# KyanChen/RSPrompter

Measured on AMD Instinct MI355X. Metric: images/sec (1024x1024 synthetic tiles, rsprompter_anchor SAM-ViT-H, full predict path), higher is better.
Workload: dtype f32 (fp32 in/out; GEMMs and attention as fp16x3 split-precision MFMA with fp32 accumulate); 1 GPU; rsprompter_anchor SAM-ViT-huge, batch 8x1024x1024 per GPU, 10 classes, seeded synthetic weights (the per-GPU slice of BASELINE.json configs[3] on 1 GPU); parallelism=single GPU

## Files before the change

### include/rsp_hip.h

```cpp
#ifndef RSP_HIP_H_
#define RSP_HIP_H_

#include <stdint.h>

#ifdef __cplusplus
extern "C" {
#endif

#define RSP_OK 0
#define RSP_EINVAL (-1)
#define RSP_ELAUNCH (-2)

#define RSP_ACT_NONE 0
#define RSP_ACT_RELU 1
#define RSP_ACT_GELU 2
#define RSP_ACT_SIGMOID 3
#define RSP_ACT_RELU_POST 4

typedef void* rsp_stream_t;

int rsp_abi_version(void);
const char* rsp_build_info(void);

#define RSP_PLANE_F8 0x100
// ... 100 lines not shown
  int64_t k_bs, k_ts, k_hs;
  int64_t v_bs, v_ts, v_hs;
  int64_t o_bs, o_ts, o_hs;
  int32_t B, nh, dh, Tq, Tk;
  float scale;
  uint16_t* out_hi; uint16_t* out_lo; int32_t out_scale_log2;
  const uint8_t* mask;
} RspAttnDesc;
int rsp_attention(const RspAttnDesc* desc, rsp_stream_t stream);

int rsp_sam_t2i_attention(const float* q, const float* kv, const int32_t* kv_map, float* out, int32_t R, int32_t T,
                          int32_t N, float scale, rsp_stream_t stream);
int rsp_sam_i2t_attention(const float* q, const int32_t* q_map, const float* k, const float* v, float* out,
                          uint16_t* out_hi, uint16_t* out_lo, int32_t out_scale_log2, int32_t R, int32_t T, int32_t N,
                          float scale, rsp_stream_t stream);
typedef struct RspI2tFusedDesc {
  const float* q; const int32_t* q_map; const float* k; const float* v;
  const float* wo; const float* bo;
  const float* res; const int32_t* res_map;
  const uint16_t* res_hi; const uint16_t* res_lo; int32_t res_scale_log2;
  const float* gamma; const float* beta; float eps;
  float* out; uint16_t* out_hi; uint16_t* out_lo; int32_t out_scale_log2;
  int32_t R, T, N; float scale;
} RspI2tFusedDesc;
int rsp_sam_i2t_fused(const RspI2tFusedDesc* desc, rsp_stream_t stream);

typedef struct RspRoiAlignDesc {
  const float* feat[4];
  const float* pe[4];
  int32_t H[4], W[4];
  float spatial_scale[4];
  const float* rois;
  float* out;
  int32_t K, P, C, num_levels, finest_scale;
} RspRoiAlignDesc;
int rsp_roi_align(const RspRoiAlignDesc* desc, rsp_stream_t stream);

typedef struct RspBoxCoder {
  float means[4], stds[4];
  float max_ratio;
  float ctr_clamp;
  int32_t clip_border;
  int32_t add_ctr_clamp;
} RspBoxCoder;
typedef struct RspRpnDesc {
  const float* head[5];
// ... 163 lines not shown
```

### rsprompter_amd/_lib.py

```python
import ctypes
import os

_HERE = os.path.dirname(os.path.abspath(__file__))
LIB_PATH = os.path.join(_HERE, "librsp_hip.so")

c_void_p = ctypes.c_void_p
c_int = ctypes.c_int
c_int64 = ctypes.c_int64
c_float = ctypes.c_float


class RspGemmDesc(ctypes.Structure):
    _fields_ = [
        ("A", c_void_p), ("Bhi", c_void_p), ("Blo", c_void_p), ("C", c_void_p),
        ("bias", c_void_p), ("res", c_void_p), ("a_rowmap", c_void_p), ("c_rowmap", c_void_p),
        ("M", c_int), ("N", c_int), ("K", c_int),
        ("lda", c_int), ("ldc", c_int), ("ldr", c_int),
        ("res_mod", c_int), ("act", c_int),
        ("alpha", c_float), ("a_scale_log2", c_int),
        ("conv_k", c_int), ("conv_stride", c_int), ("conv_pad", c_int),
        ("conv_H", c_int), ("conv_W", c_int), ("conv_C", c_int),
        ("conv_Ho", c_int), ("conv_Wo", c_int),
        ("ct_W", c_int), ("ct_dy", c_int),
        ("res_bmap", c_void_p), ("res_brows", c_int),
# ... 14 lines not shown
        ("q_bs", c_int64), ("q_ts", c_int64), ("q_hs", c_int64),
        ("k_bs", c_int64), ("k_ts", c_int64), ("k_hs", c_int64),
        ("v_bs", c_int64), ("v_ts", c_int64), ("v_hs", c_int64),
        ("o_bs", c_int64), ("o_ts", c_int64), ("o_hs", c_int64),
        ("B", c_int), ("nh", c_int), ("dh", c_int), ("Tq", c_int), ("Tk", c_int),
        ("scale", c_float),
        ("out_hi", c_void_p), ("out_lo", c_void_p), ("out_scale_log2", c_int),
        ("mask", c_void_p),
    ]


class RspMaskEmbedDesc(ctypes.Structure):
    _fields_ = [(n, c_void_p) for n in (
        "mask_pred_plus", "image_embeddings", "roi_img", "conv1_w", "conv1_b", "ln1_w", "ln1_b", "conv2_w",
        "conv2_b", "ln2_w", "ln2_b", "conv3_w", "conv3_b", "out")] + [
        ("R", c_int), ("he", c_int), ("we", c_int), ("C", c_int), ("eps", c_float)]


class RspI2tFusedDesc(ctypes.Structure):
    _fields_ = [("q", c_void_p), ("q_map", c_void_p), ("k", c_void_p), ("v", c_void_p), ("wo", c_void_p), ("bo", c_void_p),
                ("res", c_void_p), ("res_map", c_void_p), ("res_hi", c_void_p), ("res_lo", c_void_p),
                ("res_scale_log2", c_int), ("gamma", c_void_p), ("beta", c_void_p), ("eps", c_float),
                ("out", c_void_p), ("out_hi", c_void_p), ("out_lo", c_void_p), ("out_scale_log2", c_int),
                ("R", c_int), ("T", c_int), ("N", c_int), ("scale", c_float)]


class RspRoiAlignDesc(ctypes.Structure):
    _fields_ = [
        ("feat", c_void_p * 4), ("pe", c_void_p * 4), ("H", c_int * 4), ("W", c_int * 4),
        ("spatial_scale", c_float * 4), ("rois", c_void_p), ("out", c_void_p),
        ("K", c_int), ("P", c_int), ("C", c_int), ("num_levels", c_int), ("finest_scale", c_int),
    ]


class RspBoxCoder(ctypes.Structure):
    _fields_ = [("means", c_float * 4), ("stds", c_float * 4), ("max_ratio", c_float), ("ctr_clamp", c_float),
                ("clip_border", c_int), ("add_ctr_clamp", c_int)]


class RspRpnDesc(ctypes.Structure):
    _fields_ = [
        ("head", c_void_p * 5), ("H", c_int * 5), ("W", c_int * 5), ("stride", c_float * 5),
        ("ld", c_int), ("A", c_int), ("nms_pre", c_int), ("num_levels", c_int),
        ("base_anchors", c_void_p), ("coder", RspBoxCoder), ("min_bbox_size", c_float),
    ]


# ... 155 lines not shown
```

### rsprompter_amd/csrc/samattn.hip

```cpp
#include <stdlib.h>
#include "rsp_common.h"

namespace {

constexpr int NH = 8, DH = 16, W = NH * DH;
constexpr float LOG2E = 1.4426950408889634f;

template <int TMAX>
__global__ __launch_bounds__(512) void sam_t2i_kernel(const float* __restrict__ q, const float* __restrict__ kv,
                                                      const int32_t* __restrict__ kv_map, float* __restrict__ out,
                                                      int T, int N, float scale) {
  constexpr int HD = DH / 2;
  __shared__ __attribute__((aligned(16))) float sQ[TMAX * W];
  const int r = blockIdx.x;
  const int tid = threadIdx.x, lane = tid & 63;
  const int h = __builtin_amdgcn_readfirstlane(tid >> 6);
  const int half = lane & 1;
  for (int i = tid; i < TMAX * W; i += 512)
    sQ[i] = (i < T * W) ? q[(int64_t)r * T * W + i] * (scale * LOG2E) : 0.f;
  __syncthreads();
  const int64_t rb = kv_map ? kv_map[r] : r;
  const float* kbase = kv + rb * (int64_t)N * (2 * W) + h * DH + half * HD;
  const float* qbase = &sQ[h * DH + half * HD];

// ... 132 lines not shown
      if (out) *reinterpret_cast<f32x4*>(out + orow * W + h * DH + 4 * c) = o[c];
      if (ohi) {
        half4_t h4, l4;
#pragma unroll
        for (int e = 0; e < 4; ++e) { half_t a, b; rsp_split1(o[c][e] * pscale, a, b); h4[e] = a; l4[e] = b; }
        const int col = h * DH + 4 * c;
        const int64_t po = ((int64_t)(col >> 5) * out_rows + orow) * 32 + (col & 31);
        *reinterpret_cast<half4_t*>(ohi + po) = h4;
        *reinterpret_cast<half4_t*>(olo + po) = l4;
      }
    }
  }
}


struct I2tFusedP {
  const float* q; const int32_t* q_map; const float* k; const float* v;
  const float* wo; const float* bo;
  const float* res; const int32_t* res_map;
  const half_t* res_hi; const half_t* res_lo; float res_inv_scale; int64_t res_rows;
  const float* gamma; const float* beta; float eps;
  float* out; half_t* ohi; half_t* olo; float pscale; int64_t out_rows;
  int T, N; float scale;
};
constexpr int FUSED_PIX_PER_BLOCK = 512, CO = 256;

template <int TMAX>
__global__ __launch_bounds__(1024) void sam_i2t_fused_kernel(const I2tFusedP p) {
  constexpr int PST = TMAX * NH + 8;
  __shared__ __attribute__((aligned(16))) float sK[TMAX * W];
  __shared__ __attribute__((aligned(16))) float sV[TMAX * W];
  __shared__ __attribute__((aligned(16))) float sVp[TMAX * NH * CO];
  __shared__ __attribute__((aligned(16))) float sP[128 * PST];
  __shared__ __attribute__((aligned(16))) float sBo[CO], sG[CO], sB[CO];
  const int r = blockIdx.y;
  const int tid = threadIdx.x;
  const int T = p.T, N = p.N;
  if (tid < CO) { sBo[tid] = p.bo[tid]; sG[tid] = p.gamma[tid]; sB[tid] = p.beta[tid]; }
  for (int i = tid; i < TMAX * W; i += 1024) {
    const bool ok = i < T * W;
    sK[i] = ok ? p.k[(int64_t)r * T * W + i] * (p.scale * LOG2E) : 0.f;
    sV[i] = ok ? p.v[(int64_t)r * T * W + i] : 0.f;
  }
  __syncthreads();
  for (int i = tid; i < TMAX * NH * CO; i += 1024) {
    const int c = i & (CO - 1), th = i >> 8, h = th & 7, t = th >> 3;
// ... 89 lines not shown
    for (int j = 0; j < 8; ++j)
#pragma unroll
      for (int e = 0; e < 4; ++e) { const float dl = acc[j][e] - mean; sq += dl * dl; }
    sq += __shfl_xor(sq, 1, 64); sq += __shfl_xor(sq, 2, 64); sq += __shfl_xor(sq, 4, 64);
    const float rstd = 1.0f / sqrtf(sq * (1.0f / CO) + p.eps);
    if (!live) continue;
#pragma unroll
    for (int j = 0; j < 8; ++j) {
      f32x4 o;
      const f32x4 g4 = *reinterpret_cast<const f32x4*>(&sG[32 * j + 4 * l8]);
      const f32x4 b4 = *reinterpret_cast<const f32x4*>(&sB[32 * j + 4 * l8]);
#pragma unroll
      for (int e = 0; e < 4; ++e) o[e] = (acc[j][e] - mean) * rstd * g4[e] + b4[e];
      if (p.out) *reinterpret_cast<f32x4*>(p.out + orow * CO + 32 * j + 4 * l8) = o;
      if (p.ohi) rsp_store_planes4(p.ohi, p.olo, ((int64_t)j * p.out_rows + orow) * 32 + 4 * l8, o * p.pscale, false);
    }
  }
}


constexpr int F2_THREADS = 512, F2_RPOS = 256, F2_POS = 1024;
typedef float f32x16_t __attribute__((ext_vector_type(16)));

template <int NKS, bool RES_F32>
__global__ __launch_bounds__(F2_THREADS) void sam_i2t_fused_mfma_kernel(const I2tFusedP p) {
  constexpr int TT = 2 * NKS;
  constexpr int TBR = 272, TBW = 32 * TBR, PGB = NKS * 2 * 1024;
  constexpr int REG = PGB > TBW ? PGB : TBW;
  __shared__ __attribute__((aligned(1024))) unsigned char smem[8 * REG + (2 * TT * W + 3 * CO + 2 * 8 * 8 * 32 + 16) * 4];
  float* const sK = reinterpret_cast<float*>(smem + 8 * REG);
  float* const sV = sK + TT * W;
  float* const sBo = sV + TT * W;
  float* const sG = sBo + CO;
  float* const sB = sG + CO;
  float* const sSum = sB + CO;
  float* const sSq = sSum + 8 * 8 * 32;
  float* const sRed = sSq + 8 * 8 * 32;
  const int r = blockIdx.y;
  const int tid = threadIdx.x, lane = tid & 63;
  const int wave = __builtin_amdgcn_readfirstlane(tid >> 6);
  const int hh = lane >> 5, l31 = lane & 31;
  const int T = p.T, N = p.N;
  if (tid < CO) { sBo[tid] = p.bo[tid]; sG[tid] = p.gamma[tid]; sB[tid] = p.beta[tid]; }
  for (int i = tid; i < TT * W; i += F2_THREADS) {
    const bool ok = i < T * W;
    sK[i] = ok ? p.k[(int64_t)r * T * W + i] * (p.scale * LOG2E) : 0.f;
    sV[i] = ok ? p.v[(int64_t)r * T * W + i] : 0.f;
  }
  __syncthreads();
  half8_t ah[NKS], al[NKS];
  float unscale;
  {
    float vp[NKS][8];
// ... 19 lines not shown
    }
    vmax = rsp_wave_max(vmax);
    if (lane == 0) sRed[wave] = vmax;
    __syncthreads();
    float bm = sRed[0];
#pragma unroll
    for (int w = 1; w < 8; ++w) bm = fmaxf(bm, sRed[w]);
    int ve = 0;
    if (bm > 0.f) { int ex; frexpf(bm, &ex); ve = 13 - ex; }
    ve = max(-24, min(24, ve));
    const float vs = ldexpf(1.0f, ve);
    unscale = ldexpf(1.0f, -(14 + ve));
#pragma unroll
    for (int s_ = 0; s_ < NKS; ++s_)
#pragma unroll
      for (int h = 0; h < 8; ++h) {
        half_t a, b;
        rsp_split1(vp[s_][h] * vs, a, b);
        ah[s_][h] = a; al[s_][h] = b;
      }
  }
  const int64_t qb = p.q_map ? p.q_map[r] : r;
  const int64_t rb = p.res_map ? p.res_map[r] : r;
  unsigned char* const piece = smem + wave * REG;
  const int p_blk = blockIdx.x * F2_POS;
  const int lr0 = lane >> 4, c4 = (lane & 15) * 4;
  const int ch0 = wave * 32 + 4 * hh;

  for (int rd = 0; rd < F2_POS / F2_RPOS; ++rd) {
    const int p_round = p_blk + rd * F2_RPOS;
    if (p_round >= N) break;
    asm volatile("" ::: "memory");
    {
      const int p_base = p_round + wave * 32;
      unsigned char* const tb_row = piece + lr0 * TBR + c4 * 4;
      unsigned char* const tb_pos = piece + l31 * TBR;
      float sc[NKS][8];
#pragma unroll
      for (int half = 0; half < 2; ++half) {
#pragma unroll
        for (int g = 0; g < 8; ++g) {
          const int pos = min(p_base + g * 4 + lr0, N - 1);
          const f32x4 x = *reinterpret_cast<const f32x4*>(p.q + (qb * N + pos) * (int64_t)W + half * 64 + c4);
          *reinterpret_cast<f32x4*>(tb_row + g * 4 * TBR) = x;
        }
        RSP_WAVE_LOCKSTEP();
#pragma unroll
        for (int hl = 0; hl < 4; ++hl) {
          const int h = half * 4 + hl;
          f32x4 qv[4];
#pragma unroll
          for (int u = 0; u < 4; ++u) qv[u] = *reinterpret_cast<const f32x4*>(tb_pos + (hl * 4 + u) * 16);
#pragma unroll
          for (int tt = 0; tt < NKS; ++tt) {
            const float* kr = sK + (2 * tt + hh) * W + h * DH;
            f32x2 a2 = {0.f, 0.f};
// ... 12 lines not shown
#pragma unroll
      for (int h = 0; h < 8; ++h) {
        float m = sc[0][h];
#pragma unroll
        for (int tt = 1; tt < NKS; ++tt) m = fmaxf(m, sc[tt][h]);
        m = fmaxf(m, __shfl_xor(m, 32, 64));
        float sm = 0.f;
#pragma unroll
        for (int tt = 0; tt < NKS; ++tt) { sc[tt][h] = __builtin_amdgcn_exp2f(sc[tt][h] - m); sm += sc[tt][h]; }
        sm += __shfl_xor(sm, 32, 64);
        const float inv = 16384.0f / sm;
#pragma unroll
        for (int tt = 0; tt < NKS; ++tt) sc[tt][h] *= inv;
      }
#pragma unroll
      for (int tt = 0; tt < NKS; ++tt) {
        half8_t ph, pl;
        rsp_split8_trunc(sc[tt], ph, pl);
        *reinterpret_cast<half8_t*>(piece + (tt * 2 + 0) * 1024 + lane * 16) = ph;
        *reinterpret_cast<half8_t*>(piece + (tt * 2 + 1) * 1024 + lane * 16) = pl;
      }
    }
    __syncthreads();
#pragma unroll 1
    for (int g0 = 0; g0 < 8; g0 += 4) {
    f32x16_t acc[4];
#pragma unroll
    for (int gl = 0; gl < 4; ++gl) {
      const int g = g0 + gl;
#pragma unroll
      for (int e = 0; e < 16; ++e) acc[gl][e] = 0.f;
#pragma unroll
      for (int s_ = 0; s_ < NKS; ++s_) {
        const half8_t bh = *reinterpret_cast<const half8_t*>(smem + g * REG + (s_ * 2 + 0) * 1024 + lane * 16);
        const half8_t bl = *reinterpret_cast<const half8_t*>(smem + g * REG + (s_ * 2 + 1) * 1024 + lane * 16);
        acc[gl] = __builtin_amdgcn_mfma_f32_32x32x16_f16(al[s_], bh, acc[gl], 0, 0, 0);
        acc[gl] = __builtin_amdgcn_mfma_f32_32x32x16_f16(ah[s_], bl, acc[gl], 0, 0, 0);
        acc[gl] = __builtin_amdgcn_mfma_f32_32x32x16_f16(ah[s_], bh, acc[gl], 0, 0, 0);
      }
      __builtin_amdgcn_sched_barrier(0);
    }
    f32x4 rf[2][4];
    half4_t rh[2][4], rl[2][4];
    auto res_load = [&](int g, int b) {
      const int pos = min(p_round + g * 32 + l31, N - 1);
      if constexpr (RES_F32) {
        const float* rp = p.res + (rb * N + pos) * (int64_t)CO + ch0;
#pragma unroll
        for (int a = 0; a < 4; ++a) rf[b][a] = *reinterpret_cast<const f32x4*>(rp + 8 * a);
      } else {
        const int64_t ro = ((int64_t)wave * p.res_rows + (int64_t)r * N + pos) * 32 + 4 * hh;
#pragma unroll
        for (int a = 0; a < 4; ++a) {
          rh[b][a] = *reinterpret_cast<const half4_t*>(p.res_hi + ro + 8 * a);
          rl[b][a] = *reinterpret_cast<const half4_t*>(p.res_lo + ro + 8 * a);
        }
      }
    };
// ... 81 lines not shown
}

extern "C" int rsp_sam_i2t_attention(const float* q, const int32_t* q_map, const float* k, const float* v, float* out,
                                     uint16_t* out_hi, uint16_t* out_lo, int32_t out_scale_log2, int32_t R, int32_t T,
                                     int32_t N, float scale, rsp_stream_t stream) {
  if (!q || !k || !v || (!out && !(out_hi && out_lo)) || R < 0 || T <= 0 || T > 16 || N <= 0) return RSP_EINVAL;
  if ((out_hi == nullptr) != (out_lo == nullptr)) return RSP_EINVAL;
  if (R == 0) return RSP_OK;
  if (R > 65535) return RSP_EINVAL;
  hipStream_t s = (hipStream_t)stream;
  dim3 grid((N + PIX_PER_BLOCK - 1) / PIX_PER_BLOCK, R);
  half_t* hi = reinterpret_cast<half_t*>(out_hi);
  half_t* lo = reinterpret_cast<half_t*>(out_lo);
  const float ps = ldexpf(1.0f, out_scale_log2);
  const int64_t rows = (int64_t)R * N;
  if (T <= 8) hipLaunchKernelGGL((sam_i2t_kernel<8>), grid, dim3(256), 0, s, q, q_map, k, v, out, hi, lo, ps, T, N, rows, scale);
  else if (T <= 12) hipLaunchKernelGGL((sam_i2t_kernel<12>), grid, dim3(256), 0, s, q, q_map, k, v, out, hi, lo, ps, T, N, rows, scale);
  else hipLaunchKernelGGL((sam_i2t_kernel<16>), grid, dim3(256), 0, s, q, q_map, k, v, out, hi, lo, ps, T, N, rows, scale);
  RSP_CHECK_LAUNCH();
  return RSP_OK;
}

extern "C" int rsp_sam_i2t_fused(const RspI2tFusedDesc* d, rsp_stream_t stream) {
  if (!d || !d->q || !d->k || !d->v || !d->wo || !d->bo || !d->gamma || !d->beta) return RSP_EINVAL;
  if (!d->out && !(d->out_hi && d->out_lo)) return RSP_EINVAL;
  if ((d->out_hi == nullptr) != (d->out_lo == nullptr)) return RSP_EINVAL;
  if ((d->res != nullptr) == (d->res_hi != nullptr) || (d->res_hi && !d->res_lo)) return RSP_EINVAL;
  if (d->R < 0 || d->T <= 0 || d->T > 10 || d->N <= 0 || d->R > 65535) return RSP_EINVAL;
  if (RSP_PLANE_IS_F8(d->out_scale_log2) || RSP_PLANE_IS_F8(d->res_scale_log2)) return RSP_EINVAL;
  if (d->R == 0) return RSP_OK;
  I2tFusedP p;
  p.q = d->q; p.q_map = d->q_map; p.k = d->k; p.v = d->v; p.wo = d->wo; p.bo = d->bo;
  p.res = d->res; p.res_map = d->res_map;
  p.res_hi = reinterpret_cast<const half_t*>(d->res_hi); p.res_lo = reinterpret_cast<const half_t*>(d->res_lo);
  p.res_inv_scale = ldexpf(1.0f, -RSP_PLANE_EXP(d->res_scale_log2)); p.res_rows = (int64_t)d->R * d->N;
  p.gamma = d->gamma; p.beta = d->beta; p.eps = d->eps;
  p.out = d->out; p.ohi = reinterpret_cast<half_t*>(d->out_hi); p.olo = reinterpret_cast<half_t*>(d->out_lo);
  p.pscale = ldexpf(1.0f, RSP_PLANE_EXP(d->out_scale_log2)); p.out_rows = (int64_t)d->R * d->N;
  p.T = d->T; p.N = d->N; p.scale = d->scale;
  hipStream_t s = (hipStream_t)stream;
  const bool mfma_form = !d->out;
  if (mfma_form) {
    dim3 grid2((d->N + F2_POS - 1) / F2_POS, d->R);
    const bool f32res = d->res != nullptr;
    if (d->T <= 8) {
      if (f32res) hipLaunchKernelGGL((sam_i2t_fused_mfma_kernel<4, true>), grid2, dim3(F2_THREADS), 0, s, p);
      else hipLaunchKernelGGL((sam_i2t_fused_mfma_kernel<4, false>), grid2, dim3(F2_THREADS), 0, s, p);
    } else {
      if (f32res) hipLaunchKernelGGL((sam_i2t_fused_mfma_kernel<5, true>), grid2, dim3(F2_THREADS), 0, s, p);
      else hipLaunchKernelGGL((sam_i2t_fused_mfma_kernel<5, false>), grid2, dim3(F2_THREADS), 0, s, p);
    }
    RSP_CHECK_LAUNCH();
    return RSP_OK;
  }
  dim3 grid((d->N + FUSED_PIX_PER_BLOCK - 1) / FUSED_PIX_PER_BLOCK, d->R);
  if (d->T <= 8) hipLaunchKernelGGL((sam_i2t_fused_kernel<8>), grid, dim3(1024), 0, s, p);
  else hipLaunchKernelGGL((sam_i2t_fused_kernel<10>), grid, dim3(1024), 0, s, p);
  RSP_CHECK_LAUNCH();
  return RSP_OK;
}
```

### rsprompter_amd/ops.py

```python
import math
import os

import torch

from . import _lib as _lib_real

ACT_NONE, ACT_RELU, ACT_GELU, ACT_SIGMOID, ACT_RELU_POST = 0, 1, 2, 3, 4
DEFAULT_A_SCALE_LOG2 = 2
DEBUG_FINITE = bool(int(__import__('os').environ.get('RSP_DEBUG_FINITE', '0')))


class Profiler:

    def __init__(self):
        self.records = []

    def summary(self):
        torch.cuda.synchronize()
        agg = {}
        for name, flops, nbytes, e0, e1 in self.records:
            a = agg.setdefault(name, dict(ms=0.0, calls=0, flops=0.0, bytes=0.0))
            a['ms'] += e0.elapsed_time(e1)
            a['calls'] += 1
            a['flops'] += flops
# ... 393 lines not shown


def vit_window_attention(q, kv, rel_tab, Bp, nh, dh, scale, planes=False, f8=False, win_grid=None, variant=0):
    lib = _lib.load()
    T, D = 196, nh * dh
    if not isinstance(kv, Planes) or kv.shape[-1] != 2 * D or kv.rows < Bp * T or kv.f8:
        raise ValueError('kv must be the fp16 K | V planes of the qkv GEMM')
    if tuple(rel_tab.shape) != (2, 2, 32, dh + 8) or rel_tab.dtype != torch.float16 or not rel_tab.is_contiguous():
        raise ValueError('rel_tab must come from pack_relpos_tables')
    _chk_f32(q, 'q')
    out = None if planes else torch.empty((Bp * T, D), dtype=torch.float32, device=q.device)
    pl = empty_planes((Bp * T, D), q.device, f8=f8) if planes else None
    hi, lo, e = (pl.hi.data_ptr(), pl.lo.data_ptr(), pl.word) if planes else (0, 0, 0)
    wn, wr = (int(win_grid[0]), int(win_grid[1])) if win_grid is not None else (0, 0)
    _timed('attn_win_kernel<vit,window>', 4.0 * Bp * nh * T * T * dh, 0,
           lambda: _lib.check(lib.rsp_vit_window_attention(q.data_ptr(), q.stride(0), kv.hi.data_ptr(), kv.lo.data_ptr(),
                                                           kv.rows, kv.scale_log2, rel_tab.data_ptr(), _ptr(out), hi, lo, e,
                                                           Bp, nh, dh, scale, wn, wr, variant, _stream()),
                              'rsp_vit_window_attention'))
    return pl if planes else out


SAM_I2T_FUSED_MAX_TOKENS = 10


def sam_i2t_fused(q, k, v, wo, bo, gamma, beta, *, R, T, N, scale, eps=1e-6, q_map=None, res=None, res_map=None,
                  res_planes=None, planes=True, f32=False):
    lib = _lib.load()
    for t, n in ((q, 'q'), (k, 'k'), (v, 'v'), (wo, 'wo'), (bo, 'bo'), (gamma, 'gamma'), (beta, 'beta')):
        _chk_f32(t, n)
        if not t.is_contiguous():
            raise ValueError(f'sam_i2t_fused: {n} must be contiguous')
    if tuple(wo.shape) != (256, 128) or q.shape[-1] != 128:
        raise ValueError('sam_i2t_fused expects internal width 128 and a [256, 128] out_proj weight')
    if (res is None) == (res_planes is None):
        raise ValueError('sam_i2t_fused: exactly one of res / res_planes')
    d = _lib.RspI2tFusedDesc()
    d.q, d.q_map, d.k, d.v, d.wo, d.bo = q.data_ptr(), _ptr(q_map), k.data_ptr(), v.data_ptr(), wo.data_ptr(), bo.data_ptr()
    if res is not None:
        _chk_f32(res, 'res')
        if not res.is_contiguous() or res.shape[-1] != 256:
            raise ValueError('sam_i2t_fused: res must be contiguous rows of 256')
        d.res, d.res_map = res.data_ptr(), _ptr(res_map)
    else:
        if res_planes.f8 or res_planes.rows != R * N or res_planes.shape[-1] != 256:
            raise ValueError('sam_i2t_fused: res_planes must be the fp16 hi / lo planes of the [R*N, 256] tensor')
        d.res_hi, d.res_lo, d.res_scale_log2 = res_planes.hi.data_ptr(), res_planes.lo.data_ptr(), res_planes.scale_log2
    d.gamma, d.beta, d.eps = gamma.data_ptr(), beta.data_ptr(), eps
    out = torch.empty((R * N, 256), dtype=torch.float32, device=q.device) if f32 else None
    pl = empty_planes((R * N, 256), q.device) if planes else None
    d.out = _ptr(out)
    if pl is not None:
        d.out_hi, d.out_lo, d.out_scale_log2 = pl.hi.data_ptr(), pl.lo.data_ptr(), pl.scale_log2
    d.R, d.T, d.N, d.scale = R, T, N, scale
    _timed('sam_i2t_fused_kernel', 2.0 * R * N * T * (128 + 8 * 256), 4.0 * R * N * (128 + 256 + 256),
           lambda: _lib.check(lib.rsp_sam_i2t_fused(d, _stream()), "rsp_sam_i2t_fused"), detail=f'R={R} T={T} N={N}')
    if planes and f32:
        return out, pl
    return pl if planes else out


_attn_ws = {}


def _attn_workspace(nbytes, device):
    key = str(device)
    buf = _attn_ws.get(key)
    if buf is None or buf.numel() < nbytes:
        buf = torch.empty((nbytes,), dtype=torch.uint8, device=device)
        _attn_ws[key] = buf
    return buf


def vit_attention(qkv, rel, Bp, S, nh, dh, scale, planes=False):
    lib = _lib.load()
    kind = 'global' if S * S >= 1024 else 'window'
    fl = 4.0 * Bp * nh * (S * S) ** 2 * dh
    pl = empty_planes((Bp * S * S, nh * dh), qkv.device) if planes else None
# ... 912 lines not shown
```

### rsprompter_amd/sam_decoder.py

```python
import math

import numpy as np
import torch

from . import ops
from .nnutil import HIPModule, add_param, infer_sam_arch, nchw_view, nhwc_view
from .registry import MODELS

HID = 256
HEADS = 8
MLP_DIM = 2048
N_MASK_TOKENS = 4


def _upscale2_k_order():
    return [32 * ((kp >> 4) >> 1) + 8 * ((8 * ((kp >> 4) & 1) + (kp & 7)) >> 2) + 4 * ((kp >> 3) & 1) + (kp & 3) for kp in range(64)]


def _add_linear(root, name, cout, cin):
    add_param(root, name + '.weight', (cout, cin))
    add_param(root, name + '.bias', (cout,))


def _add_ln(root, name, c):
# ... 26 lines not shown
            _add_attn(self, p + '.cross_attn_image_to_token', HID // 2)
            for j in range(1, 5):
                _add_ln(self, f'{p}.layer_norm{j}', HID)
            _add_linear(self, p + '.mlp.lin1', MLP_DIM, HID)
            _add_linear(self, p + '.mlp.lin2', HID, MLP_DIM)
        _add_attn(self, 'transformer.final_attn_token_to_image', HID // 2)
        _add_ln(self, 'transformer.layer_norm_final_attn', HID)
        add_param(self, 'upscale_conv1.weight', (HID, HID // 4, 2, 2))
        add_param(self, 'upscale_conv1.bias', (HID // 4,))
        add_param(self, 'upscale_conv2.weight', (HID // 4, HID // 8, 2, 2))
        add_param(self, 'upscale_conv2.bias', (HID // 8,))
        _add_ln(self, 'upscale_layer_norm', HID // 4)
        for i in range(N_MASK_TOKENS):
            p = f'output_hypernetworks_mlps.{i}'
            _add_linear(self, p + '.proj_in', HID, HID)
            _add_linear(self, p + '.layers.0', HID, HID)
            _add_linear(self, p + '.proj_out', HID // 8, HID)
        _add_linear(self, 'iou_prediction_head.proj_in', HID, HID)
        _add_linear(self, 'iou_prediction_head.layers.0', HID, HID)
        _add_linear(self, 'iou_prediction_head.proj_out', N_MASK_TOKENS, HID)
        self._pe_cache = {}
        self.t2i_fold = True
        self.upscale_fused = True
        self.keep_stages = False
        self._last_stages = None
        self.max_prompt_sets = None

    def _pw(self, name, with_bias=True):
        m = _g(self, name)
        return ops.PackedWeight(m.weight, m.bias if with_bias else None)

    def _pack(self):
        from .necks import convt_weights4
        P = {}
        for i in range(2):
            p = f'transformer.layers.{i}'
            for a in ('self_attn', 'cross_attn_token_to_image', 'cross_attn_image_to_token'):
                for pr in ('q_proj', 'k_proj', 'v_proj', 'out_proj'):
                    P[f'{i}.{a}.{pr}'] = self._pw(f'{p}.{a}.{pr}')
            P[f'{i}.lin1'] = self._pw(p + '.mlp.lin1')
            P[f'{i}.lin2'] = self._pw(p + '.mlp.lin2')
        for pr in ('q_proj', 'k_proj', 'v_proj', 'out_proj'):
            P[f'final.{pr}'] = self._pw(f'transformer.final_attn_token_to_image.{pr}')
        P['up1'] = convt_weights4(self.upscale_conv1.weight, self.upscale_conv1.bias)
        P['up2'] = convt_weights4(self.upscale_conv2.weight, self.upscale_conv2.bias)
        w2 = self.upscale_conv2.weight.detach()[_upscale2_k_order()]
# ... 165 lines not shown
            keys_pl = ops.layernorm(keys, m4.weight, m4.bias, 1e-6, planes=True, f32=False)
            del keys
        del qi, kv_img

        qpe = ops.add_rows(q, tokens0)
        q = self._token_attn(qpe, qpe, q, '1.self_attn', R, T, res=q)
        q = self._ln(q, 'transformer.layers.1.layer_norm1')
        qpe = ops.add_rows(q, tokens0)
        tq = ops.gemm(qpe, P['1.cross_attn_token_to_image.q_proj'])
        fold = self.t2i_fold and T <= ops.SAM_T2I_FOLD_MAX_TOKENS and N % 32 == 0 and R * N * 512 < 2 ** 31
        kv = None
        if fold:
            ao = self._t2i_folded('1.cross_attn_token_to_image', tq, keys_pl, pe_t, R, T, N)
        else:
            kv = ops.gemm(keys_pl, P['1.cross_attn_token_to_image.kv_proj'], bias=None,
                          res=pe_t['1.cross_attn_token_to_image.kv_proj'], res_mod=N)
            self._t2i(tq, kv, ao, R, T, N)
        q = ops.gemm(ao, P['1.cross_attn_token_to_image.out_proj'], res=q)
        q = self._ln(q, 'transformer.layers.1.layer_norm2')
        hmid = ops.gemm(q, P['1.lin1'], act=ops.ACT_RELU)
        q = ops.gemm(hmid, P['1.lin2'], res=q)
        q = self._ln(q, 'transformer.layers.1.layer_norm3')
        qpe = ops.add_rows(q, tokens0)
        qi = ops.gemm(keys_pl, P['1.cross_attn_image_to_token.q_proj'], bias=None,
                      res=pe_t['1.cross_attn_image_to_token.q_proj'], res_mod=N)
        kt = ops.gemm(qpe, P['1.cross_attn_image_to_token.k_proj'])
        vt = ops.gemm(q, P['1.cross_attn_image_to_token.v_proj'])
        m4 = _g(self, 'transformer.layers.1.layer_norm4')
        if fused:
            op = _g(self, 'transformer.layers.1.cross_attn_image_to_token.out_proj')
            keys_pl = ops.sam_i2t_fused(qi, kt, vt, op.weight.detach(), op.bias.detach(), m4.weight, m4.bias, R=R, T=T,
                                        N=N, scale=dh2 ** -0.5, eps=1e-6, res_planes=keys_pl)
        else:
            self._i2t(qi, kt, vt, ai, R, T, N)
            keys = ops.gemm(ai, P['1.cross_attn_image_to_token.out_proj'], res=keys_pl)
            keys_pl = ops.layernorm(keys, m4.weight, m4.bias, 1e-6, planes=True, f32=False)
            del keys

        qpe = ops.add_rows(q, tokens0)
        tq = ops.gemm(qpe, P['final.q_proj'])
        if fold:
            ao = self._t2i_folded('final', tq, keys_pl, pe_t, R, T, N)
        else:
            kv = ops.gemm(keys_pl, P['final.kv_proj'], bias=None, res=pe_t['final.kv_proj'], res_mod=N, out=kv)
            self._t2i(tq, kv, ao, R, T, N)
        q = ops.gemm(ao, P['final.out_proj'], res=q)
        q = self._ln(q, 'transformer.layer_norm_final_attn', eps=1e-5)
        del kv, qi, ai
        q3 = q.view(R, T, HID)
        stages = dict(keys=keys_pl, tokens=q3, up=None, hyper=[]) if self.keep_stages else None

        toks = (1, 2, 3) if multimask_output else (0,)
        fused_up = self.upscale_fused and len(toks) == 1
        if not fused_up:
            up = ops.conv_transpose2x2(keys_pl.view(R, h, w, HID), *P['up1'], act=ops.ACT_GELU,
# ... 144 lines not shown
```

Before: 52.56 images/s.

## Fold image-to-token q projection into fused i2t attention kernel

Adds a QFOLD variant of the fused image-to-token MFMA kernel. It computes the q projection (keys planes times q_proj weight, plus the positional term) inside the kernel. The weight chunks are streamed through a triple-buffered LDS ring with explicit vmcnt waits. This removes a separate GEMM launch and the write and re-read of the fp32 qi tensor, at the cost of more LDS, extra MFMA work per block and a more complex pipeline that could lower occupancy.

After: 52.71 images/s (median of 6 runs). No clear change (+0.3%).

```diff
diff --git a/include/rsp_hip.h b/include/rsp_hip.h
--- a/include/rsp_hip.h
+++ b/include/rsp_hip.h
@@ -146,6 +146,8 @@
   const float* gamma; const float* beta; float eps;
   float* out; uint16_t* out_hi; uint16_t* out_lo; int32_t out_scale_log2;
   int32_t R, T, N; float scale;
+  const uint16_t* q_w_hi; const uint16_t* q_w_lo; int32_t q_w_scale_log2;
+  const float* q_pe; int32_t q_pe_mod;
 } RspI2tFusedDesc;
 int rsp_sam_i2t_fused(const RspI2tFusedDesc* desc, rsp_stream_t stream);
 
diff --git a/rsprompter_amd/_lib.py b/rsprompter_amd/_lib.py
--- a/rsprompter_amd/_lib.py
+++ b/rsprompter_amd/_lib.py
@@ -60,7 +60,8 @@
                 ("res", c_void_p), ("res_map", c_void_p), ("res_hi", c_void_p), ("res_lo", c_void_p),
                 ("res_scale_log2", c_int), ("gamma", c_void_p), ("beta", c_void_p), ("eps", c_float),
                 ("out", c_void_p), ("out_hi", c_void_p), ("out_lo", c_void_p), ("out_scale_log2", c_int),
-                ("R", c_int), ("T", c_int), ("N", c_int), ("scale", c_float)]
+                ("R", c_int), ("T", c_int), ("N", c_int), ("scale", c_float),
+                ("q_w_hi", c_void_p), ("q_w_lo", c_void_p), ("q_w_scale_log2", c_int), ("q_pe", c_void_p), ("q_pe_mod", c_int)]
 
 
 class RspRoiAlignDesc(ctypes.Structure):
diff --git a/rsprompter_amd/csrc/samattn.hip b/rsprompter_amd/csrc/samattn.hip
--- a/rsprompter_amd/csrc/samattn.hip
+++ b/rsprompter_amd/csrc/samattn.hip
@@ -1,4 +1,5 @@
 #include <stdlib.h>
+#include <type_traits>
 #include "rsp_common.h"
 
 namespace {
@@ -178,6 +179,8 @@
   const float* gamma; const float* beta; float eps;
   float* out; half_t* ohi; half_t* olo; float pscale; int64_t out_rows;
   int T, N; float scale;
+  const half_t* wq_hi; const half_t* wq_lo; float q_alpha;
+  const float* peq;
 };
 constexpr int FUSED_PIX_PER_BLOCK = 512, CO = 256;
 
@@ -313,13 +316,16 @@
 constexpr int F2_THREADS = 512, F2_RPOS = 256, F2_POS = 1024;
 typedef float f32x16_t __attribute__((ext_vector_type(16)));
 
-template <int NKS, bool RES_F32>
+template <int NKS, bool RES_F32, bool QFOLD>
 __global__ __launch_bounds__(F2_THREADS) void sam_i2t_fused_mfma_kernel(const I2tFusedP p) {
+  static_assert(!(QFOLD && RES_F32), "the q projection reads the residual PLANES");
   constexpr int TT = 2 * NKS;
   constexpr int TBR = 272, TBW = 32 * TBR, PGB = NKS * 2 * 1024;
-  constexpr int REG = PGB > TBW ? PGB : TBW;
-  __shared__ __attribute__((aligned(1024))) unsigned char smem[8 * REG + (2 * TT * W + 3 * CO + 2 * 8 * 8 * 32 + 16) * 4];
-  float* const sK = reinterpret_cast<float*>(smem + 8 * REG);
+  constexpr int REG = (QFOLD || PGB > TBW) ? PGB : TBW;
+  constexpr int WPL = W * 64, WCH = 2 * WPL, WRING = QFOLD ? 3 * WCH : 0;
+  __shared__ __attribute__((aligned(1024))) unsigned char smem[WRING + 8 * REG + (2 * TT * W + 3 * CO + 2 * 8 * 8 * 32 + 16) * 4];
+  unsigned char* const pbase = smem + WRING;
+  float* const sK = reinterpret_cast<float*>(pbase + 8 * REG);
   float* const sV = sK + TT * W;
   float* const sBo = sV + TT * W;
   float* const sG = sBo + CO;
@@ -385,16 +391,162 @@
   }
   const int64_t qb = p.q_map ? p.q_map[r] : r;
   const int64_t rb = p.res_map ? p.res_map[r] : r;
-  unsigned char* const piece = smem + wave * REG;
+  unsigned char* const piece = pbase + wave * REG;
   const int p_blk = blockIdx.x * F2_POS;
   const int lr0 = lane >> 4, c4 = (lane & 15) * 4;
   const int ch0 = wave * 32 + 4 * hh;
+
+  typedef __attribute__((address_space(3))) unsigned char* lds_u8;
+  const rsp_lds_addr_t wring = rsp_lds_addr((lds_u8)smem);
+  const int w_rho = (wave * 64 + lane) >> 2;
+  const int w_row = 16 * (2 * (w_rho >> 5) + ((w_rho >> 2) & 1)) + 4 * ((w_rho & 31) >> 3) + (w_rho & 3);
+  const int w_src = w_row * 64 + (((lane & 3) ^ ((w_rho >> 2) & 3)) << 4);
+  auto issue_w = [&](int kc, int buf) {
+    const unsigned char* sh = reinterpret_cast<const unsigned char*>(p.wq_hi) + kc * WPL + w_src;
+    const unsigned char* sl = reinterpret_cast<const unsigned char*>(p.wq_lo) + kc * WPL + w_src;
+    RSP_GLOBAL_LOAD_LDS_B128(sh, wring + (buf * WCH + wave * 1024));
+    RSP_GLOBAL_LOAD_LDS_B128(sl, wring + (buf * WCH + WPL + wave * 1024));
+  };
+  half8_t xh[4][2], xl[4][2];
+  auto load_x = [&](int p_round, int kc, half8_t (&h8)[2], half8_t (&l8)[2]) {
+    const int64_t row = (int64_t)r * N + min(p_round + wave * 32 + l31, N - 1);
+#pragma unroll
+    for (int s_ = 0; s_ < 2; ++s_) {
+      const int64_t o = ((int64_t)kc * p.res_rows + row) * 32 + 16 * s_ + 8 * hh;
+      RSP_GLOBAL_LOAD_B128(h8[s_], p.res_hi + o);
+      RSP_GLOBAL_LOAD_B128(l8[s_], p.res_lo + o);
+    }
+  };
+  auto w_head = [&]() {
+    issue_w(0, 0);
+    issue_w(1, 1);
+    __builtin_amdgcn_sched_barrier(0);
+  };
+  if constexpr (QFOLD) w_head();
 
   for (int rd = 0; rd < F2_POS / F2_RPOS; ++rd) {
     const int p_round = p_blk + rd * F2_RPOS;
     if (p_round >= N) break;
     asm volatile("" ::: "memory");
-    {
+    if constexpr (QFOLD) {
+      f32x16_t qa[4];
+#pragma unroll
+      for (int j = 0; j < 4; ++j)
+#pragma unroll
+        for (int e = 0; e < 16; ++e) qa[j][e] = 0.f;
+      load_x(p_round, 0, xh[0], xl[0]);
+      __builtin_amdgcn_sched_barrier(0);
+      load_x(p_round, 1, xh[1], xl[1]);
+      __builtin_amdgcn_sched_barrier(0);
+      load_x(p_round, 2, xh[2], xl[2]);
+      __builtin_amdgcn_sched_barrier(0);
+      auto k_step = [&](auto cc) {
+        constexpr int c = decltype(cc)::value, cur = c & 3;
+        if constexpr (c == 0) asm volatile("s_waitcnt vmcnt(8)" ::: "memory");
+        else if constexpr (c < 6) asm volatile("s_waitcnt vmcnt(10)" ::: "memory");
+        else if constexpr (c == 6) asm volatile("s_waitcnt vmcnt(6)" ::: "memory");
+        else asm volatile("s_waitcnt vmcnt(0)" ::: "memory");
+        __builtin_amdgcn_s_barrier();
+        if constexpr (c + 2 < 8) {
+          issue_w(c + 2, (c + 2) % 3);
+          __builtin_amdgcn_sched_barrier(0);
+        }
+        if constexpr (c + 3 < 8) {
+          load_x(p_round, c + 3, xh[(c + 3) & 3], xl[(c + 3) & 3]);
+          __builtin_amdgcn_sched_barrier(0);
+        }
+        const unsigned char* rdw = smem + (c % 3) * WCH;
+#pragma unroll
+        for (int s_ = 0; s_ < 2; ++s_) {
+#pragma unroll
+          for (int j0 = 0; j0 < 4; j0 += 2) {
+            half8_t wh[2], wl[2];
+#pragma unroll
+            for (int jj = 0; jj < 2; ++jj) {
+              const int wrow = (j0 + jj) * 32 + l31;
+              const int off = (wrow * 4 + ((2 * s_ + hh) ^ ((wrow >> 2) & 3))) * 16;
+              wh[jj] = *reinterpret_cast<const half8_t*>(rdw + off);
+              wl[jj] = *reinterpret_cast<const half8_t*>(rdw + WPL + off);
+            }
+#pragma unroll
+            for (int jj = 0; jj < 2; ++jj)
+              qa[j0 + jj] = __builtin_amdgcn_mfma_f32_32x32x16_f16(wh[jj], xl[cur][s_], qa[j0 + jj], 0, 0, 0);
+#pragma unroll
+            for (int jj = 0; jj < 2; ++jj)
+              qa[j0 + jj] = __builtin_amdgcn_mfma_f32_32x32x16_f16(wl[jj], xh[cur][s_], qa[j0 + jj], 0, 0, 0);
+#pragma unroll
+            for (int jj = 0; jj < 2; ++jj)
+              qa[j0 + jj] = __builtin_amdgcn_mfma_f32_32x32x16_f16(wh[jj], xh[cur][s_], qa[j0 + jj], 0, 0, 0);
+          }
+        }
+      };
+      k_step(std::integral_constant<int, 0>{});
+      k_step(std::integral_constant<int, 1>{});
+      k_step(std::integral_constant<int, 2>{});
+      k_step(std::integral_constant<int, 3>{});
+      k_step(std::integral_constant<int, 4>{});
+      k_step(std::integral_constant<int, 5>{});
+      k_step(std::integral_constant<int, 6>{});
+      k_step(std::integral_constant<int, 7>{});
+      const float* peq = p.peq + (int64_t)min(p_round + wave * 32 + l31, N - 1) * W + 16 * hh;
+      float pr[4][TT];
+#pragma unroll
+      for (int j = 0; j < 4; ++j) {
+        f32x4 qv[4];
+#pragma unroll
+        for (int u = 0; u < 4; ++u) {
+          const f32x4 pe4 = *reinterpret_cast<const f32x4*>(peq + 32 * j + 4 * u);
+          {
+#pragma clang fp contract(off)
+#pragma unroll
+            for (int e = 0; e < 4; ++e) {
+              const float y = qa[j][4 * u + e] * p.q_alpha + 0.f;
+              qv[u][e] = y + pe4[e];
+            }
+          }
+        }
+        const float* kh = sK + (2 * j + hh) * DH;
+        float mx = -INFINITY;
+#pragma unroll
+        for (int t = 0; t < TT; ++t) {
+          const float* kr = kh + t * W;
+          f32x2 a2 = {0.f, 0.f};
+#pragma unroll
+          for (int u = 0; u < 4; ++u) {
+            const f32x4 kk = *reinterpret_cast<const f32x4*>(kr + 4 * u);
+            a2 = __builtin_elementwise_fma(f32x2{qv[u][0], qv[u][1]}, f32x2{kk[0], kk[1]}, a2);
+            a2 = __builtin_elementwise_fma(f32x2{qv[u][2], qv[u][3]}, f32x2{kk[2], kk[3]}, a2);
+          }
+          pr[j][t] = (t < T) ? a2[0] + a2[1] : -INFINITY;
+          mx = fmaxf(mx, pr[j][t]);
+        }
+        float se = 0.f, so = 0.f;
+#pragma unroll
+        for (int t = 0; t < TT; t += 2) {
+          pr[j][t] = __builtin_amdgcn_exp2f(pr[j][t] - mx); se += pr[j][t];
+          pr[j][t + 1] = __builtin_amdgcn_exp2f(pr[j][t + 1] - mx); so += pr[j][t + 1];
+        }
+        const float inv = 16384.0f / (se + so);
+#pragma unroll
+        for (int t = 0; t < TT; ++t) pr[j][t] *= inv;
+        __builtin_amdgcn_sched_barrier(0);
+      }
+#pragma unroll
+      for (int s_ = 0; s_ < NKS; ++s_) {
+        float fr[8];
+#pragma unroll
+        for (int j = 0; j < 4; ++j) {
+          const float own = hh ? pr[j][2 * s_ + 1] : pr[j][2 * s_];
+          const float oth = __shfl_xor(hh ? pr[j][2 * s_] : pr[j][2 * s_ + 1], 32, 64);
+          fr[2 * j] = hh ? oth : own;
+          fr[2 * j + 1] = hh ? own : oth;
+        }
+        half8_t ph, pl;
+        rsp_split8_trunc(fr, ph, pl);
+        *reinterpret_cast<half8_t*>(piece + (s_ * 2 + 0) * 1024 + lane * 16) = ph;
+        *reinterpret_cast<half8_t*>(piece + (s_ * 2 + 1) * 1024 + lane * 16) = pl;
+      }
+    } else {
       const int p_base = p_round + wave * 32;
       unsigned char* const tb_row = piece + lr0 * TBR + c4 * 4;
       unsigned char* const tb_pos = piece + l31 * TBR;
@@ -453,6 +605,9 @@
       }
     }
     __syncthreads();
+    if constexpr (QFOLD) {
+      if (rd + 1 < F2_POS / F2_RPOS && p_round + F2_RPOS < N) w_head();
+    }
 #pragma unroll 1
     for (int g0 = 0; g0 < 8; g0 += 4) {
     f32x16_t acc[4];
@@ -463,8 +618,8 @@
       for (int e = 0; e < 16; ++e) acc[gl][e] = 0.f;
 #pragma unroll
       for (int s_ = 0; s_ < NKS; ++s_) {
-        const half8_t bh = *reinterpret_cast<const half8_t*>(smem + g * REG + (s_ * 2 + 0) * 1024 + lane * 16);
-        const half8_t bl = *reinterpret_cast<const half8_t*>(smem + g * REG + (s_ * 2 + 1) * 1024 + lane * 16);
+        const half8_t bh = *reinterpret_cast<const half8_t*>(pbase + g * REG + (s_ * 2 + 0) * 1024 + lane * 16);
+        const half8_t bl = *reinterpret_cast<const half8_t*>(pbase + g * REG + (s_ * 2 + 1) * 1024 + lane * 16);
         acc[gl] = __builtin_amdgcn_mfma_f32_32x32x16_f16(al[s_], bh, acc[gl], 0, 0, 0);
         acc[gl] = __builtin_amdgcn_mfma_f32_32x32x16_f16(ah[s_], bl, acc[gl], 0, 0, 0);
         acc[gl] = __builtin_amdgcn_mfma_f32_32x32x16_f16(ah[s_], bh, acc[gl], 0, 0, 0);
@@ -592,7 +747,11 @@
 }
 
 extern "C" int rsp_sam_i2t_fused(const RspI2tFusedDesc* d, rsp_stream_t stream) {
-  if (!d || !d->q || !d->k || !d->v || !d->wo || !d->bo || !d->gamma || !d->beta) return RSP_EINVAL;
+  if (!d || !d->k || !d->v || !d->wo || !d->bo || !d->gamma || !d->beta) return RSP_EINVAL;
+  const bool qfold = !d->q;
+  if (qfold && (!d->q_w_hi || !d->q_w_lo || !d->q_pe || !d->res_hi || d->res || d->out || d->q_map || d->q_pe_mod != d->N ||
+                RSP_PLANE_IS_F8(d->q_w_scale_log2)))
+    return RSP_EINVAL;
   if (!d->out && !(d->out_hi && d->out_lo)) return RSP_EINVAL;
   if ((d->out_hi == nullptr) != (d->out_lo == nullptr)) return RSP_EINVAL;
   if ((d->res != nullptr) == (d->res_hi != nullptr) || (d->res_hi && !d->res_lo)) return RSP_EINVAL;
@@ -608,17 +767,26 @@
   p.out = d->out; p.ohi = reinterpret_cast<half_t*>(d->out_hi); p.olo = reinterpret_cast<half_t*>(d->out_lo);
   p.pscale = ldexpf(1.0f, RSP_PLANE_EXP(d->out_scale_log2)); p.out_rows = (int64_t)d->R * d->N;
   p.T = d->T; p.N = d->N; p.scale = d->scale;
+  p.wq_hi = p.wq_lo = nullptr; p.q_alpha = 0.f; p.peq = nullptr;
+  if (qfold) {
+    p.wq_hi = reinterpret_cast<const half_t*>(d->q_w_hi); p.wq_lo = reinterpret_cast<const half_t*>(d->q_w_lo);
+    p.q_alpha = ldexpf(1.0f, -(RSP_PLANE_EXP(d->res_scale_log2) + RSP_PLANE_EXP(d->q_w_scale_log2)));
+    p.peq = d->q_pe;
+  }
   hipStream_t s = (hipStream_t)stream;
   const bool mfma_form = !d->out;
   if (mfma_form) {
     dim3 grid2((d->N + F2_POS - 1) / F2_POS, d->R);
     const bool f32res = d->res != nullptr;
-    if (d->T <= 8) {
-      if (f32res) hipLaunchKernelGGL((sam_i2t_fused_mfma_kernel<4, true>), grid2, dim3(F2_THREADS), 0, s, p);
-      else hipLaunchKernelGGL((sam_i2t_fused_mfma_kernel<4, false>), grid2, dim3(F2_THREADS), 0, s, p);
+    if (qfold) {
+      if (d->T <= 8) hipLaunchKernelGGL((sam_i2t_fused_mfma_kernel<4, false, true>), grid2, dim3(F2_THREADS), 0, s, p);
+      else hipLaunchKernelGGL((sam_i2t_fused_mfma_kernel<5, false, true>), grid2, dim3(F2_THREADS), 0, s, p);
+    } else if (d->T <= 8) {
+      if (f32res) hipLaunchKernelGGL((sam_i2t_fused_mfma_kernel<4, true, false>), grid2, dim3(F2_THREADS), 0, s, p);
+      else hipLaunchKernelGGL((sam_i2t_fused_mfma_kernel<4, false, false>), grid2, dim3(F2_THREADS), 0, s, p);
     } else {
-      if (f32res) hipLaunchKernelGGL((sam_i2t_fused_mfma_kernel<5, true>), grid2, dim3(F2_THREADS), 0, s, p);
-      else hipLaunchKernelGGL((sam_i2t_fused_mfma_kernel<5, false>), grid2, dim3(F2_THREADS), 0, s, p);
+      if (f32res) hipLaunchKernelGGL((sam_i2t_fused_mfma_kernel<5, true, false>), grid2, dim3(F2_THREADS), 0, s, p);
+      else hipLaunchKernelGGL((sam_i2t_fused_mfma_kernel<5, false, false>), grid2, dim3(F2_THREADS), 0, s, p);
     }
     RSP_CHECK_LAUNCH();
     return RSP_OK;
diff --git a/rsprompter_amd/ops.py b/rsprompter_amd/ops.py
--- a/rsprompter_amd/ops.py
+++ b/rsprompter_amd/ops.py
@@ -439,21 +439,37 @@
 
 
 SAM_I2T_FUSED_MAX_TOKENS = 10
+SAM_I2T_QPROJ = True
 
 
 def sam_i2t_fused(q, k, v, wo, bo, gamma, beta, *, R, T, N, scale, eps=1e-6, q_map=None, res=None, res_map=None,
-                  res_planes=None, planes=True, f32=False):
-    lib = _lib.load()
-    for t, n in ((q, 'q'), (k, 'k'), (v, 'v'), (wo, 'wo'), (bo, 'bo'), (gamma, 'gamma'), (beta, 'beta')):
+                  res_planes=None, planes=True, f32=False, q_weight=None, q_pe=None):
+    lib = _lib.load()
+    qfold = q is None
+    chk = [(k, 'k'), (v, 'v'), (wo, 'wo'), (bo, 'bo'), (gamma, 'gamma'), (beta, 'beta')]
+    chk.append((q_pe, 'q_pe') if qfold and q_pe is not None else (q, 'q'))
+    if qfold:
+        if q_weight is None or q_pe is None:
+            raise ValueError('sam_i2t_fused: q, or q_weight and q_pe')
+        if getattr(q_weight, 'f8', False) or (q_weight.N, q_weight.K) != (128, 256) or tuple(q_pe.shape) != (N, 128):
+            raise ValueError('sam_i2t_fused: q_weight must be the fp16 planes of a [128, 256] weight, q_pe [N, 128]')
+        if res_planes is None or q_map is not None or f32 or not planes:
+            raise ValueError('sam_i2t_fused: the q-projecting form takes res_planes, no q_map, and writes planes only')
+    elif q_weight is not None or q_pe is not None:
+        raise ValueError('sam_i2t_fused: q_weight / q_pe replace q')
+    for t, n in chk:
         _chk_f32(t, n)
         if not t.is_contiguous():
             raise ValueError(f'sam_i2t_fused: {n} must be contiguous')
-    if tuple(wo.shape) != (256, 128) or q.shape[-1] != 128:
+    if tuple(wo.shape) != (256, 128) or (not qfold and q.shape[-1] != 128):
         raise ValueError('sam_i2t_fused expects internal width 128 and a [256, 128] out_proj weight')
     if (res is None) == (res_planes is None):
         raise ValueError('sam_i2t_fused: exactly one of res / res_planes')
     d = _lib.RspI2tFusedDesc()
-    d.q, d.q_map, d.k, d.v, d.wo, d.bo = q.data_ptr(), _ptr(q_map), k.data_ptr(), v.data_ptr(), wo.data_ptr(), bo.data_ptr()
+    d.q, d.q_map, d.k, d.v, d.wo, d.bo = _ptr(q), _ptr(q_map), k.data_ptr(), v.data_ptr(), wo.data_ptr(), bo.data_ptr()
+    if qfold:
+        d.q_w_hi, d.q_w_lo, d.q_w_scale_log2 = q_weight.hi.data_ptr(), q_weight.lo.data_ptr(), q_weight.scale_log2
+        d.q_pe, d.q_pe_mod = q_pe.data_ptr(), N
     if res is not None:
         _chk_f32(res, 'res')
         if not res.is_contiguous() or res.shape[-1] != 256:
@@ -464,13 +480,16 @@
             raise ValueError('sam_i2t_fused: res_planes must be the fp16 hi / lo planes of the [R*N, 256] tensor')
         d.res_hi, d.res_lo, d.res_scale_log2 = res_planes.hi.data_ptr(), res_planes.lo.data_ptr(), res_planes.scale_log2
     d.gamma, d.beta, d.eps = gamma.data_ptr(), beta.data_ptr(), eps
-    out = torch.empty((R * N, 256), dtype=torch.float32, device=q.device) if f32 else None
-    pl = empty_planes((R * N, 256), q.device) if planes else None
+    dev = k.device
+    out = torch.empty((R * N, 256), dtype=torch.float32, device=dev) if f32 else None
+    pl = empty_planes((R * N, 256), dev) if planes else None
     d.out = _ptr(out)
     if pl is not None:
         d.out_hi, d.out_lo, d.out_scale_log2 = pl.hi.data_ptr(), pl.lo.data_ptr(), pl.scale_log2
     d.R, d.T, d.N, d.scale = R, T, N, scale
-    _timed('sam_i2t_fused_kernel', 2.0 * R * N * T * (128 + 8 * 256), 4.0 * R * N * (128 + 256 + 256),
+    flops = 2.0 * R * N * T * (128 + 8 * 256) + (2.0 * R * N * 256 * 128 if qfold else 0.0)
+    nbytes = 4.0 * R * N * ((0 if qfold else 128) + 256 + 256)
+    _timed('sam_i2t_fused_kernel<qproj>' if qfold else 'sam_i2t_fused_kernel', flops, nbytes,
            lambda: _lib.check(lib.rsp_sam_i2t_fused(d, _stream()), "rsp_sam_i2t_fused"), detail=f'R={R} T={T} N={N}')
     if planes and f32:
         return out, pl
diff --git a/rsprompter_amd/sam_decoder.py b/rsprompter_amd/sam_decoder.py
--- a/rsprompter_amd/sam_decoder.py
+++ b/rsprompter_amd/sam_decoder.py
@@ -72,6 +72,7 @@
         self._pe_cache = {}
         self.t2i_fold = True
         self.upscale_fused = True
+        self.i2t_fold_q = True
         self.keep_stages = False
         self._last_stages = None
         self.max_prompt_sets = None
@@ -283,15 +284,20 @@
         q = ops.gemm(hmid, P['1.lin2'], res=q)
         q = self._ln(q, 'transformer.layers.1.layer_norm3')
         qpe = ops.add_rows(q, tokens0)
-        qi = ops.gemm(keys_pl, P['1.cross_attn_image_to_token.q_proj'], bias=None,
-                      res=pe_t['1.cross_attn_image_to_token.q_proj'], res_mod=N)
+        fold_q = self.i2t_fold_q and fused and getattr(ops, 'SAM_I2T_QPROJ', False)
+        qi = None
+        if not fold_q:
+            qi = ops.gemm(keys_pl, P['1.cross_attn_image_to_token.q_proj'], bias=None,
+                          res=pe_t['1.cross_attn_image_to_token.q_proj'], res_mod=N)
         kt = ops.gemm(qpe, P['1.cross_attn_image_to_token.k_proj'])
         vt = ops.gemm(q, P['1.cross_attn_image_to_token.v_proj'])
         m4 = _g(self, 'transformer.layers.1.layer_norm4')
         if fused:
             op = _g(self, 'transformer.layers.1.cross_attn_image_to_token.out_proj')
+            qarg = dict(q_weight=P['1.cross_attn_image_to_token.q_proj'],
+                        q_pe=pe_t['1.cross_attn_image_to_token.q_proj']) if fold_q else {}
             keys_pl = ops.sam_i2t_fused(qi, kt, vt, op.weight.detach(), op.bias.detach(), m4.weight, m4.bias, R=R, T=T,
-                                        N=N, scale=dh2 ** -0.5, eps=1e-6, res_planes=keys_pl)
+                                        N=N, scale=dh2 ** -0.5, eps=1e-6, res_planes=keys_pl, **qarg)
         else:
             self._i2t(qi, kt, vt, ai, R, T, N)
             keys = ops.gemm(ai, P['1.cross_attn_image_to_token.out_proj'], res=keys_pl)
```
